# RIKEN-RCCS/EigenExa

Measured on AMD Instinct MI355X. Metric: eigen_sx full-solve throughput (reference flop model: 4/3 N^3 + D&C GEMM + 2 nvec N^2), higher is better.
Workload: dtype f64; 1 GPU; N=8192 random symmetric fp64 (counter-based R+R^T, seed 20240807), eigen_sx all eigenpairs, m_forward=64, m_backward=128; parallelism=1 GPU (1x1 grid)

## Files before the change

eigenexa_amd/csrc/api.hip:

```cpp
#include "eigx_context.h"
#include "eigx_comm.h"
#include "../../include/eigenexa_amd.h"
#include <cstring>

namespace eigx {
Context g_ctx;
}

using namespace eigx;

extern "C" {

int eigx_init(int device) {
  return eigx_init_multi(device, 0, 1, nullptr, 'C');
}

int eigx_get_device_count(void) {
  int ndev = 0;
  if (hipGetDeviceCount(&ndev) != hipSuccess) { (void)hipGetLastError(); return 0; }
  return ndev;
}

int eigx_get_rccl_unique_id(void* out128) {
  return comm_get_unique_id(out128);
// ... 245 lines not shown
int eigx_profile_read(double* out6) {
  if (!g_ctx.initialized) return EIGX_ERR_NOT_INITIALIZED;
  if (!out6) return EIGX_ERR_BAD_ARG;
  EIGX_HIP_CHECK(hipSetDevice(g_ctx.device));
  EIGX_HIP_CHECK(hipStreamSynchronize(g_ctx.stream));
  for (int q = 0; q < 6; ++q) out6[q] = 0.0;
  for (size_t q = 0; q < g_ctx.prof_kind.size(); ++q) {
    float ms = 0.f;
    EIGX_HIP_CHECK(hipEventElapsedTime(&ms, g_ctx.prof_ev[2 * q], g_ctx.prof_ev[2 * q + 1]));
    if (g_ctx.prof_kind[q] > 1) continue;
    const int k = g_ctx.prof_kind[q] ? 3 : 0;
    out6[k + 0] += 1.0;
    out6[k + 1] += g_ctx.prof_units[q];
    out6[k + 2] += 1e-3 * ms;
  }
  return EIGX_OK;
}

int eigx_profile_read_kinds(double* out, int nkinds) {
  if (!g_ctx.initialized) return EIGX_ERR_NOT_INITIALIZED;
  if (!out || nkinds < 1) return EIGX_ERR_BAD_ARG;
  EIGX_HIP_CHECK(hipSetDevice(g_ctx.device));
  EIGX_HIP_CHECK(hipStreamSynchronize(g_ctx.stream));
  for (int q = 0; q < 3 * nkinds; ++q) out[q] = 0.0;
  for (size_t q = 0; q < g_ctx.prof_kind.size(); ++q) {
    const int k = g_ctx.prof_kind[q];
    if (k < 0 || k >= nkinds) continue;
    float ms = 0.f;
    EIGX_HIP_CHECK(hipEventElapsedTime(&ms, g_ctx.prof_ev[2 * q], g_ctx.prof_ev[2 * q + 1]));
    out[3 * k + 0] += 1.0;
    out[3 * k + 1] += g_ctx.prof_units[q];
    out[3 * k + 2] += 1e-3 * ms;
  }
  return EIGX_OK;
}

int eigx_device_synchronize(void) {
  if (!g_ctx.initialized) return EIGX_ERR_NOT_INITIALIZED;
  EIGX_HIP_CHECK(hipSetDevice(g_ctx.device));
  EIGX_HIP_CHECK(hipDeviceSynchronize());
  return EIGX_OK;
}

void* eigx_malloc_dev(int64_t bytes) {
  if (!g_ctx.initialized) return nullptr;
  void* p = nullptr;
  if (hipMalloc(&p, (size_t)bytes) != hipSuccess) return nullptr;
  return p;
}
int eigx_free_dev(void* p) {
  if (p) EIGX_HIP_CHECK(hipFree(p));
  return EIGX_OK;
}
int eigx_memcpy_h2d(void* dst, const void* src, int64_t bytes) {
  EIGX_HIP_CHECK(hipMemcpy(dst, src, (size_t)bytes, hipMemcpyHostToDevice));
  return EIGX_OK;
}
int eigx_memcpy_d2h(void* dst, const void* src, int64_t bytes) {
  EIGX_HIP_CHECK(hipMemcpy(dst, src, (size_t)bytes, hipMemcpyDeviceToHost));
  return EIGX_OK;
}

int eigx_tune(int key, int value) {
  if (key == 0) return set_gemm_variant(value);
  if (key == 1) return set_bisect_threads(value);
  if (key == 2) return set_bt_q(value);
  if (key == 3 || key == 4 || key == 5 || key == 10 || key == 11) return set_reduce_knob(key, value);
  if (key == 12) return (value >= 0 && value <= 2) ? set_reduce_knob(key, value) : -1;
  if (key == 6) return set_gemm_cstream(value);
  if (key == 7) return value > 0 ? set_reduce_knob(key, value) : -1;
  if (key == 8) return set_dc_chunk(value);
  if (key == 9) return comm_set_bounce(value);
  if (key == 15) return set_dc_pipe(value);
  if (key == 16) return set_dc_batch(value);
  if (key == 17 || key == 18 || key == 19) return set_range_knob(key, value);
  if (key == 20) return set_tri_nb(value);
  if (key == 21) return set_batch_nmax(value);
  if (key == 22) return set_hbatch_nmax(value);
  if (key == 23) return set_gbatch_nmax(value);
  if (key == 24) return set_hgbatch_nmax(value);
  if (key == 25) return set_gemm_latec_kmax(value);
  if (key == 26) return set_batch_range_route(value);
  if (key == 27) return set_batch_range_accept(value);
  return -1;
}

int eigx_dgemm_dev(char opa, char opb, int m, int n, int k, double alpha, const double* a, int lda,
                   const double* b, int ldb, double beta, double* c, int ldc, int tri_upper) {
  if (!g_ctx.initialized) return EIGX_ERR_NOT_INITIALIZED;
  EIGX_HIP_CHECK(hipStreamSynchronize(nullptr));
  dgemm_dev(g_ctx.stream, opa, opb, m, n, k, alpha, a, lda, b, ldb, beta, c, ldc, tri_upper ? 1 : 0,
            &g_ctx.grid);
  EIGX_HIP_CHECK(hipStreamSynchronize(g_ctx.stream));
  return EIGX_OK;
}

int eigx_dgemm_gather_dev(char opa, char opb, int m, int n, int k, double alpha, const double* a, int lda,
                          const double* b, int ldb, double beta, double* c, int ldc, const int* kmap_a,
                          const int* kmap_b) {
  if (!g_ctx.initialized) return EIGX_ERR_NOT_INITIALIZED;
  EIGX_HIP_CHECK(hipStreamSynchronize(nullptr));
  dgemm_dev(g_ctx.stream, opa, opb, m, n, k, alpha, a, lda, b, ldb, beta, c, ldc, 0, nullptr, kmap_a, nullptr, 1, 0,
            0, 0, 1, 0, 0, 0, 1, 0, kmap_b);
  EIGX_HIP_CHECK(hipStreamSynchronize(g_ctx.stream));
  return EIGX_OK;
}

}
```

eigenexa_amd/csrc/dc.hip:

```cpp
#include "eigx_context.h"
#include "eigx_comm.h"
#include "../../include/eigenexa_amd.h"
#include <algorithm>
#include <cfloat>
#include <cstring>

namespace eigx {

namespace {

constexpr int LEAF = 32;

constexpr int LEAF_T = 64;
__global__ __launch_bounds__(LEAF_T) void jacobi_leaf_kernel(const double* __restrict__ d,
                                                             const double* __restrict__ e, int lde, int band,
                                                             const int* __restrict__ leaf_off,
                                                             const int* __restrict__ leaf_n, double* __restrict__ D,
                                                             double* __restrict__ Q, int ldq, int r0, int r1) {
  __shared__ double A[LEAF][LEAF + 1];
  __shared__ double V[LEAF][LEAF + 1];
  __shared__ double cs[LEAF / 2][2];
  __shared__ int pq[LEAF / 2][2];
  __shared__ int perm[LEAF];
  const int tid = threadIdx.x;
// ... 172 lines not shown
  const MergeDev M = md[blockIdx.z];
  const int K = M.K;
  if ((int)(blockIdx.x * 64) >= K || (int)(blockIdx.y * ZN_IC) >= K) return;
  const int i0 = blockIdx.y * ZN_IC;
  const int i1 = (i0 + ZN_IC < K) ? i0 + ZN_IC : K;
  {
    const int i = i0 + threadIdx.x;
    double y = 0.0;
    if (i < i1) {
      const double* col = Qa + (size_t)nd[M.off + i] * ldq;
      for (int t = 0; t < M.zr_n; ++t) y += M.zr_w[t] * col[M.zr_row[t]];
    }
    ys[threadIdx.x] = y;
  }
  __syncthreads();
  const int lane = threadIdx.x & 63, wave = threadIdx.x >> 6;
  const int j = blockIdx.x * 64 + lane;
  const bool act = j < K;
  const double* Sp = S + (size_t)M.off * lds + M.off + j;
  double acc = 0.0;
  if (act)
    for (int i = i0 + wave; i < i1; i += 4) acc += ys[i - i0] * Sp[(size_t)i * lds];
  part[wave][lane] = acc;
  __syncthreads();
  if (wave == 0 && act)
    zp[(size_t)blockIdx.y * ldn + M.off + j] = (part[0][lane] + part[1][lane]) + (part[2][lane] + part[3][lane]);
}
__global__ void znext2_kernel(const MergeDev* __restrict__ md, const int* __restrict__ dsrc, const double* __restrict__ Qa,
                              int ldq, const double* __restrict__ zp, int ldn, double* __restrict__ z) {
  const MergeDev M = md[blockIdx.y];
  const int jj = blockIdx.x * blockDim.x + threadIdx.x;
  if (jj >= M.nm) return;
  double v = 0.0;
  if (jj < M.K) {
    const int nch = (M.K + ZN_IC - 1) / ZN_IC;
    for (int c = 0; c < nch; ++c) v += zp[(size_t)c * ldn + M.off + jj];
  } else {
    const double* col = Qa + (size_t)dsrc[M.off + jj] * ldq;
    for (int t = 0; t < M.zr_n; ++t) v += M.zr_w[t] * col[M.zr_row[t]];
  }
  z[M.off + jj] = v;
}

__global__ void pack_rows_kernel(const double* __restrict__ Q, int ldq, int n, int r0, int nr, int rp,
                                 double* __restrict__ out) {
  const int j = blockIdx.y;
  for (int r = blockIdx.x * blockDim.x + threadIdx.x; r < rp; r += gridDim.x * blockDim.x)
    out[(size_t)j * rp + r] = (r < nr) ? Q[(size_t)j * ldq + r0 + r] : 0.0;
}
__global__ void unpack_rows_kernel(const double* __restrict__ in, int n, int rp, double* __restrict__ Q, int ldq) {
  const int j = blockIdx.y, q = blockIdx.z;
  const double* src = in + (size_t)q * rp * n + (size_t)j * rp;
  for (int r = blockIdx.x * blockDim.x + threadIdx.x; r < rp; r += gridDim.x * blockDim.x)
    if (q * rp + r < n) Q[(size_t)j * ldq + q * rp + r] = src[r];
}

template <int CTRL>
__device__ __forceinline__ double dc_dpp_add(double v) {
  const int lo2 = __builtin_amdgcn_update_dpp(0, __double2loint(v), CTRL, 0xf, 0xf, true);
  const int hi2 = __builtin_amdgcn_update_dpp(0, __double2hiint(v), CTRL, 0xf, 0xf, true);
  return v + __hiloint2double(hi2, lo2);
}

__device__ __forceinline__ double dc_swapadd16(double v) {
  const auto lo = __builtin_amdgcn_permlane16_swap(__double2loint(v), __double2loint(v), false, false);
  const auto hi = __builtin_amdgcn_permlane16_swap(__double2hiint(v), __double2hiint(v), false, false);
  return __hiloint2double(hi[0], lo[0]) + __hiloint2double(hi[1], lo[1]);
}

__device__ __forceinline__ double group8_sum(double v) {
  v = dc_dpp_add<0xB1>(v);
  v = dc_dpp_add<0x4E>(v);
  v = dc_dpp_add<0x141>(v);
  return v;
}

template <int LPR>
__device__ __forceinline__ double group_sum(double v) {
  v = group8_sum(v);
  if (LPR == 32) { v = dc_dpp_add<0x140>(v); v = dc_swapadd16(v); }
  return v;
}

template <int LPR>
__global__ __launch_bounds__(256) void secular_kernel(const MergeDev* __restrict__ md,
                                                      const double* __restrict__ dlam,
                                                      const double* __restrict__ wz, double* __restrict__ Dn,
                                                      double* __restrict__ S, int lds, int P, int rank,
                                                      double* __restrict__ sec, int nsec) {
  const MergeDev M = md[blockIdx.y];
  const int K = M.K;
  constexpr int RPW = 256 / LPR;
  __shared__ double so[RPW], stau[RPW];
  const int jbase = (P > 1) ? (int)((long)K * rank / P) : 0;
  const int jend = (P > 1) ? (int)((long)K * (rank + 1) / P) : K;
  if (jbase + (int)(blockIdx.x * RPW) >= jend) return;
  const int sub = threadIdx.x & (LPR - 1);
  const int jraw = jbase + blockIdx.x * RPW + threadIdx.x / LPR;
  const bool act = jraw < jend;
  const int j = act ? jraw : K - 1;
  const double* __restrict__ d = dlam + M.off;
  const double* __restrict__ z = wz + M.off;
  double* Sp = S + (size_t)M.off * lds + M.off;
  const double rho = M.rho, rhoinv = 1.0 / rho;
  const double eps = DBL_EPSILON / 2.0;
  if (K == 1) {
    if (threadIdx.x == 0) {
      const double t = rho * z[0] * z[0];
      if (sec) { sec[M.off] = d[0] + t; sec[nsec + M.off] = d[0]; sec[2 * nsec + M.off] = t; }
      else { Dn[M.off] = d[0] + t; Sp[0] = -t; }
    }
    return;
  }
  const bool last = (j == K - 1);
  const int jl = last ? K - 2 : j, jr = jl + 1;
  double origin, lo, hi, tau;
  {
    const double gap = last ? rho : d[j + 1] - d[j];
    const double base = last ? d[K - 1] : d[j], half = 0.5 * gap;
    double c = 0.0;
    for (int i = sub; i < K; i += LPR)
      if (i != jl && i != jr) c += z[i] * z[i] / ((d[i] - base) - half);
    c = group_sum<LPR>(c) + rhoinv;
    const double zl2 = z[jl] * z[jl], zr2 = z[jr] * z[jr];
    const double fmid = c + zl2 / ((d[jl] - base) - half) + zr2 / ((d[jr] - base) - half);
    int org;
    if (last) { org = K - 1; if (fmid <= 0.0) { lo = 0.5 * gap; hi = gap; } else { lo = 0.0; hi = 0.5 * gap; } }
    else if (fmid > 0.0) { org = j; lo = 0.0; hi = 0.5 * gap; }
    else { org = j + 1; lo = -0.5 * gap; hi = 0.0; }
    origin = d[org];
    const double dl = d[jl] - origin, dr = d[jr] - origin;
    const double qa = c, qb = -(c * (dl + dr) + zl2 + zr2), qc = c * dl * dr + zl2 * dr + zr2 * dl;
    tau = 0.5 * (lo + hi);
    const double disc = qb * qb - 4.0 * qa * qc;
    if (disc >= 0.0) {
      const double sq = sqrt(disc);
      const double qq = -0.5 * (qb + (qb >= 0.0 ? sq : -sq));
      const double r1 = (qa != 0.0) ? qq / qa : NAN, r2 = (qq != 0.0) ? qc / qq : NAN;
      if (r1 > lo && r1 < hi) tau = r1;
      else if (r2 > lo && r2 < hi) tau = r2;
    }
  }
  for (int iter = 0; iter < 100; ++iter) {
    double psi = 0.0, dpsi = 0.0, phi = 0.0, dphi = 0.0, err = 0.0;
    for (int i = sub; i < K; i += LPR) {
      const double t = z[i] / ((d[i] - origin) - tau);
      const double zt = z[i] * t, tt = t * t;
      if (i <= jl) { psi += zt; dpsi += tt; err += fabs(psi); }
      else { phi += zt; dphi += tt; err += fabs(phi); }
    }
    psi = group_sum<LPR>(psi); dpsi = group_sum<LPR>(dpsi);
    phi = group_sum<LPR>(phi); dphi = group_sum<LPR>(dphi);
    err = group_sum<LPR>(err);
    const double wv = rhoinv + phi + psi;
    err = 8.0 * (fabs(phi) + fabs(psi)) + err + 2.0 * rhoinv + fabs(tau) * (dpsi + dphi);
    if (fabs(wv) <= eps * err) break;
    if (wv < 0.0) lo = tau; else hi = tau;
    const double Dl = (d[jl] - origin) - tau, Dr = (d[jr] - origin) - tau;
    const double aa = (Dl + Dr) * wv - Dl * Dr * (dpsi + dphi);
    const double bb = Dl * Dr * wv;
    const double cc = wv - Dl * dpsi - Dr * dphi;
    double eta;
    {
      double disc = aa * aa - 4.0 * bb * cc;
      if (disc < 0.0) disc = 0.0;
      const double sq = sqrt(disc);
      if (cc == 0.0) eta = (aa != 0.0) ? bb / aa : 0.0;
      else if (aa <= 0.0) eta = (aa - sq) / (2.0 * cc);
      else eta = 2.0 * bb / (aa + sq);
    }
    if (wv * eta >= 0.0) eta = -wv / (dpsi + dphi);
    double tnew = tau + eta;
    if (!(tnew > lo && tnew < hi)) tnew = 0.5 * (lo + hi);
    if (tnew == tau) break;
    tau = tnew;
  }
  if (sec) {
    if (sub == 0 && act) { sec[M.off + j] = origin + tau; sec[nsec + M.off + j] = origin; sec[2 * nsec + M.off + j] = tau; }
    return;
  }
  if (sub == 0) { so[threadIdx.x / LPR] = origin; stau[threadIdx.x / LPR] = tau; if (act) Dn[M.off + j] = origin + tau; }
  __syncthreads();
  {
    const int r = threadIdx.x % RPW, ii = threadIdx.x / RPW;
    const int jr = blockIdx.x * RPW + r;
    if (jr < K) {
      const double o_ = so[r], t_ = stau[r];
      for (int i = ii; i < K; i += 256 / RPW) Sp[jr + (size_t)i * lds] = (d[i] - o_) - t_;
    }
  }
}

__global__ __launch_bounds__(256) void loewner_kernel(const MergeDev* __restrict__ md,
                                                      const double* __restrict__ dlam,
                                                      const double* __restrict__ wz, const double* __restrict__ S,
                                                      int lds, double* __restrict__ zh) {
  const MergeDev M = md[blockIdx.y];
  const int K = M.K;
  const int lane = threadIdx.x & 63;
  const int i = blockIdx.x * 4 + (threadIdx.x >> 6);
  if (i >= K) return;
  const double* d = dlam + M.off;
  const double* Sp = S + (size_t)M.off * lds + M.off + (size_t)i * lds;
  const double di = d[i];
  double prod = 1.0;
  for (int j = lane; j < K; j += 64) {
    const double num = -Sp[j];
    prod *= (j == i) ? num : num / (d[j] - di);
  }
  for (int o = 32; o > 0; o >>= 1) prod *= __shfl_xor(prod, o, 64);
  if (lane == 0) {
    const double v = sqrt(fabs(prod));
    zh[M.off + i] = (wz[M.off + i] >= 0.0) ? v : -v;
  }
}

constexpr int VEC_IC = 256;
__global__ __launch_bounds__(256) void vectors1_kernel(const MergeDev* __restrict__ md, const double* __restrict__ zh,
                                                       double* __restrict__ S, int lds, double* __restrict__ vnp,
                                                       int ldn) {
  __shared__ double part[4][64];
  const MergeDev M = md[blockIdx.z];
  const int K = M.K;
  if ((int)(blockIdx.x * 64) >= K || (int)(blockIdx.y * VEC_IC) >= K) return;
  const int lane = threadIdx.x & 63, wave = threadIdx.x >> 6;
  const int j = blockIdx.x * 64 + lane;
  const bool act = j < K;
  double* Sp = S + (size_t)M.off * lds + M.off + j;
  const double* zz = zh + M.off;
  const int i0 = blockIdx.y * VEC_IC;
  const int i1 = (i0 + VEC_IC < K) ? i0 + VEC_IC : K;
  double nrm = 0.0;
  if (act)
    for (int i = i0 + wave; i < i1; i += 4) {
      const double v = zz[i] / Sp[(size_t)i * lds];
      Sp[(size_t)i * lds] = v;
      nrm += v * v;
    }
  part[wave][lane] = nrm;
  __syncthreads();
  if (wave == 0 && act)
    vnp[(size_t)blockIdx.y * ldn + M.off + j] = (part[0][lane] + part[1][lane]) + (part[2][lane] + part[3][lane]);
}
__global__ __launch_bounds__(256) void vectors2_kernel(const MergeDev* __restrict__ md, double* __restrict__ S, int lds,
                                                       const double* __restrict__ vnp, int ldn) {
  const MergeDev M = md[blockIdx.z];
  const int K = M.K;
  if ((int)(blockIdx.x * 64) >= K || (int)(blockIdx.y * VEC_IC) >= K) return;
  const int lane = threadIdx.x & 63, wave = threadIdx.x >> 6;
  const int j = blockIdx.x * 64 + lane;
  if (j >= K) return;
  const int nch = (K + VEC_IC - 1) / VEC_IC;
  double nrm = 0.0;
  for (int c = 0; c < nch; ++c) nrm += vnp[(size_t)c * ldn + M.off + j];
  const double sc = 1.0 / sqrt(nrm);
  double* Sp = S + (size_t)M.off * lds + M.off + j;
  const int i0 = blockIdx.y * VEC_IC;
  const int i1 = (i0 + VEC_IC < K) ? i0 + VEC_IC : K;
  for (int i = i0 + wave; i < i1; i += 4) Sp[(size_t)i * lds] *= sc;
}

__global__ void scatter_lambda_kernel(const MergeDev* __restrict__ md, const double* __restrict__ sec, double* __restrict__ Dn) {
  const MergeDev M = md[blockIdx.y];
  const int j = blockIdx.x * blockDim.x + threadIdx.x;
  if (j < M.K) Dn[M.off + j] = sec[M.off + j];
}
__global__ __launch_bounds__(256) void loewner_mg_kernel(const MergeDev* __restrict__ md, const double* __restrict__ dlam,
                                                         const double* __restrict__ wz, const double* __restrict__ sec,
                                                         int nsec, double* __restrict__ zh) {
  const MergeDev M = md[blockIdx.y];
  const int K = M.K;
  const int lane = threadIdx.x & 63;
  const int i = blockIdx.x * 4 + (threadIdx.x >> 6);
  if (i >= K) return;
  const double* d = dlam + M.off;
  const double* org = sec + nsec + M.off;
  const double* tau = sec + 2 * nsec + M.off;
  const double di = d[i];
  double prod = 1.0;
  for (int j = lane; j < K; j += 64) {
    const double num = (org[j] - di) + tau[j];
    prod *= (j == i) ? num : num / (d[j] - di);
  }
  for (int o = 32; o > 0; o >>= 1) prod *= __shfl_xor(prod, o, 64);
  if (lane == 0) {
    const double v = sqrt(fabs(prod));
    zh[M.off + i] = (wz[M.off + i] >= 0.0) ? v : -v;
  }
}
__global__ __launch_bounds__(256) void vectors_mg_kernel(const MergeDev* __restrict__ md, int mi0, const double* __restrict__ dlam,
                                                         const double* __restrict__ zh, const double* __restrict__ sec, int nsec,
                                                         int j0, int j1, int compact, double* __restrict__ Sc, int ldsc) {
  __shared__ double part[4][64];
  const MergeDev M = md[mi0 + blockIdx.z];
  const int K = M.K;
  const int jhi = (j1 < K) ? j1 : K;
  const int lane = threadIdx.x & 63, wave = threadIdx.x >> 6;
  const int j = j0 + blockIdx.x * 64 + lane;
  if (j0 + (int)(blockIdx.x * 64) >= jhi) return;
  const bool act = j < jhi;
  const double* d = dlam + M.off;
  const double* zz = zh + M.off;
  const double oj = act ? sec[nsec + M.off + j] : 0.0, tj = act ? sec[2 * nsec + M.off + j] : 1.0;
  double nrm = 0.0;
  for (int i = wave; i < K; i += 4) {
    const double v = zz[i] / ((d[i] - oj) - tj);
    nrm += v * v;
  }
  part[wave][lane] = nrm;
  __syncthreads();
  const double sc = 1.0 / sqrt((part[0][lane] + part[1][lane]) + (part[2][lane] + part[3][lane]));
  if (!act) return;
  double* dst = Sc + (compact ? (size_t)M.off * ldsc : 0) + (j - j0);
  for (int i = wave; i < K; i += 4) dst[(size_t)i * ldsc] = zz[i] / ((d[i] - oj) - tj) * sc;
}

__global__ void pack_q_for_cols_kernel(const int* __restrict__ perm, const double* __restrict__ Q, int ldq, int r0, int nr,
                                       int rp, int zc, int nvec, double* __restrict__ send) {
  const int c = blockIdx.y, p = blockIdx.z;
  const int g = p * zc + c;
  if (c >= zc) return;
  double* dst = send + ((size_t)p * zc + c) * rp;
  if (g >= nvec) { for (int r = blockIdx.x * blockDim.x + threadIdx.x; r < rp; r += gridDim.x * blockDim.x) dst[r] = 0.0; return; }
  const double* src = Q + (size_t)perm[g] * ldq + r0;
  for (int r = blockIdx.x * blockDim.x + threadIdx.x; r < rp; r += gridDim.x * blockDim.x) dst[r] = (r < nr) ? src[r] : 0.0;
}
__global__ void unpack_cols_kernel(const double* __restrict__ recv, int rp, int zc, int n, double* __restrict__ Z, int ldz) {
  const int c = blockIdx.y, q = blockIdx.z;
  const double* src = recv + ((size_t)q * zc + c) * rp;
  for (int r = blockIdx.x * blockDim.x + threadIdx.x; r < rp; r += gridDim.x * blockDim.x)
    if (q * rp + r < n) Z[(size_t)c * ldz + q * rp + r] = __hip_atomic_load(src + r, __ATOMIC_RELAXED, __HIP_MEMORY_SCOPE_SYSTEM);
}

__global__ void copycols_kernel(const int* __restrict__ src, const int* __restrict__ dst,
                                const int* __restrict__ row0, const int* __restrict__ nrows,
                                const double* __restrict__ Qa, double* __restrict__ Qb, int ldq) {
  const int p = blockIdx.x;
  const double* s = Qa + (size_t)src[p] * ldq + row0[p];
  double* t = Qb + (size_t)dst[p] * ldq + row0[p];
  for (int r = threadIdx.x; r < nrows[p]; r += blockDim.x) t[r] = s[r];
}

__global__ void final_permute_kernel(const int* __restrict__ perm, const double* __restrict__ Q, int ldq, int n,
// ... 38 lines not shown

struct HostDC {
  int n, band, lde;
  std::vector<double> d, e;
  std::vector<Node> nodes;
  double& E(int i, int b) { return e[(size_t)(b - 1) * lde + i]; }

  int build(int off, int nn) {
    const int id = (int)nodes.size();
    nodes.push_back(Node());
    nodes[id].off = off; nodes[id].n = nn;
    if (nn <= LEAF) return id;
    const int n1 = nn / 2;
    nodes[id].n1 = n1;
    double c[4] = {0, 0, 0, 0}, sig[2] = {0, 0}, x[4] = {0, 0, 0, 0}, y[4] = {0, 0, 0, 0};
    for (int r = 0; r < band; ++r)
      for (int cc = r; cc < band; ++cc) {
        const int gi = off + n1 + r, gj = off + n1 - band + cc;
        c[r + band * cc] = E(gi, gi - gj);
      }
    svd2(band, c, sig, x, y);
    for (int k = 0; k < band; ++k) {
      for (int r = 0; r < band; ++r)
        for (int cc = 0; cc < band; ++cc) {
          const int i1 = off + n1 - band + r, j1 = off + n1 - band + cc;
          const double v1 = sig[k] * y[band * k + r] * y[band * k + cc];
          if (i1 == j1) d[i1] -= v1; else if (i1 < j1) E(j1, j1 - i1) -= v1;
          const int i2 = off + n1 + r, j2 = off + n1 + cc;
          const double v2 = sig[k] * x[band * k + r] * x[band * k + cc];
          if (i2 == j2) d[i2] -= v2; else if (i2 < j2) E(j2, j2 - i2) -= v2;
        }
      nodes[id].sig[k] = sig[k];
      for (int r = 0; r < band; ++r) {
        nodes[id].wv[k][r] = y[band * k + r];
        nodes[id].wv[k][band + r] = x[band * k + r];
      }
    }
    const int l = build(off, n1);
    const int r = build(off + n1, nn - n1);
    nodes[id].left = l; nodes[id].right = r;
    nodes[l].parent = id; nodes[r].parent = id;
    nodes[id].height = 1 + std::max(nodes[l].height, nodes[r].height);
    return id;
  }
};

void sort_index_runs(const double* d, int nm, std::vector<int>& idx, std::vector<int>& tmp, std::vector<int>& bounds) {
  idx.resize(nm);
  for (int i = 0; i < nm; ++i) idx[i] = i;
  bounds.clear();
  bounds.push_back(0);
  for (int i = 1; i < nm; ++i)
    if (d[i] < d[i - 1]) bounds.push_back(i);
  bounds.push_back(nm);
  auto cmp = [d](int a, int b) { return d[a] < d[b] || (d[a] == d[b] && a < b); };
  int nr = (int)bounds.size() - 1;
  if (nr > 16) { std::sort(idx.begin(), idx.end(), cmp); return; }
  tmp.resize(nm);
  while (nr > 1) {
    int w = 0;
    for (int r = 0; r < nr; r += 2) {
      if (r + 1 < nr)
        std::merge(idx.begin() + bounds[r], idx.begin() + bounds[r + 1], idx.begin() + bounds[r + 1], idx.begin() + bounds[r + 2],
                   tmp.begin() + bounds[r], cmp);
      else
        std::copy(idx.begin() + bounds[r], idx.begin() + bounds[r + 1], tmp.begin() + bounds[r]);
      bounds[w++] = bounds[r];
    }
    bounds[w] = nm;
    nr = w;
    idx.swap(tmp);
  }
}

}

int g_dc_pipe = 1, g_dc_batch = 1, g_dc_side_min = 1024;
int set_dc_pipe(int v) {
  const int old = g_dc_pipe;
  if (v >= 2) g_dc_side_min = v; else g_dc_pipe = v ? 1 : 0;
  return old;
}
int set_dc_batch(int v) { const int old = g_dc_batch; g_dc_batch = v ? 1 : 0; return old; }
int g_dc_chunk = 2048;
int set_dc_chunk(int v) {
  const int old = g_dc_chunk;
  if (v >= 64 && v <= 2048 && v % 64 == 0) g_dc_chunk = v;
  return old;
}

void band_dc_prepare(Context& ctx, int n) {
  const int P = ctx.grid.nranks;
  const int ldq = (P > 1) ? pad_ld((n + P - 1) / P + 2) : pad_ld(n);
  double* Qa = ctx.pool.get_t<double>("dc.Qa", (size_t)ldq * n);
  double* Qb = ctx.pool.get_t<double>("dc.Qb", (size_t)ldq * n);
  EIGX_HIP_CHECK(hipMemsetAsync(Qa, 0, (size_t)ldq * n * 8, ctx.side_stream));
  EIGX_HIP_CHECK(hipMemsetAsync(Qb, 0, (size_t)ldq * n * 8, ctx.side_stream));
  EIGX_HIP_CHECK(hipEventRecord(ctx.dc_ev, ctx.side_stream));
  ctx.dc_zero_n = n; ctx.dc_zero_qa = Qa; ctx.dc_zero_qb = Qb;
}

void band_dc_dev(Context& ctx, int n, int nvec, const double* d_dev, const double* e_dev, int lde, int band,
                 double* w_dev, double* z_dev, int ldz, const std::function<void()>& side_work) {
  hipStream_t st = ctx.stream;
  const double eps = DBL_EPSILON / 2.0;
  const int P = ctx.grid.nranks;
  const int rp = (n + P - 1) / P;
  const int r0 = P > 1 ? std::min(n, ctx.grid.rank * rp) : 0;
  const int r1 = P > 1 ? std::min(n, r0 + rp) : n;
  auto clip = [&](int lo, int hi, int& a, int& b) { a = std::max(lo, r0); b = std::min(hi, r1); return b > a; };
  HostDC H;
  H.n = n; H.band = band; H.lde = lde;
  H.d.resize(n);
  H.e.resize((size_t)lde * band);
  EIGX_HIP_CHECK(hipMemcpyAsync(H.d.data(), d_dev, (size_t)n * 8, hipMemcpyDeviceToHost, st));
  EIGX_HIP_CHECK(hipMemcpyAsync(H.e.data(), e_dev, (size_t)lde * band * 8, hipMemcpyDeviceToHost, st));
  EIGX_HIP_CHECK(hipStreamSynchronize(st));
  double nrm = 0.0;
  for (int i = 0; i < n; ++i) {
    nrm = std::max(nrm, fabs(H.d[i]));
    for (int b = 1; b <= band; ++b) if (i >= b) nrm = std::max(nrm, fabs(H.E(i, b)));
  }
  const double scl = nrm > 0.0 ? 1.0 / nrm : 1.0;
  for (int i = 0; i < n; ++i) {
    H.d[i] *= scl;
    for (int b = 1; b <= band; ++b) H.E(i, b) = (i >= b) ? H.E(i, b) * scl : 0.0;
  }
  H.nodes.reserve(2 * (n / (LEAF / 2) + 2));
  const int root = H.build(0, n);
  const int maxh = H.nodes[root].height;

  const bool pipe = (P == 1) && g_dc_pipe;
  const int ldq = (P > 1) ? pad_ld(rp + 2) : pad_ld(n);
  double* Qa_base = ctx.pool.get_t<double>("dc.Qa", (size_t)ldq * n);
  double* Qb_base = ctx.pool.get_t<double>("dc.Qb", (size_t)ldq * n);
  double* Qa = Qa_base - r0;
  double* Qb = Qb_base - r0;
  const int SCW = g_dc_chunk;
  const int lds_mg = SCW;
  double* Sbuf[2];
  Sbuf[0] = ctx.pool.get_t<double>("dc.S", (P > 1) ? (size_t)n * SCW + 64 : (size_t)ldq * n);
  Sbuf[1] = pipe ? ctx.pool.get_t<double>("dc.S2", (size_t)ldq * n) : Sbuf[0];
  double* sec = (P > 1) ? ctx.pool.get_t<double>("dc.sec", (size_t)3 * n) : nullptr;
  double* dd = ctx.pool.get_t<double>("dc.d", (size_t)n);
  double* de = ctx.pool.get_t<double>("dc.e", (size_t)lde * band);
  double* zh = ctx.pool.get_t<double>("dc.zh", (size_t)n);
  double* vnp = ctx.pool.get_t<double>("dc.vnp", (size_t)n * ((n + VEC_IC - 1) / VEC_IC + 1));
  double* zp = pipe ? ctx.pool.get_t<double>("dc.zp", (size_t)n * ((n + ZN_IC - 1) / ZN_IC + 1)) : nullptr;
  const int maxmerge = n / (LEAF / 2) + 8;
  int* leafinfo = ctx.pool.get_t<int>("dc.leaf", (size_t)2 * maxmerge);
  int* perm_dev = ctx.pool.get_t<int>("dc.perm", (size_t)n);
  int* iota_dev = ctx.pool.get_t<int>("dc.iota", (size_t)n);
  struct Arena {
    char *dev, *host;
    MergeDev *md_dev, *md_h;
    GemmBatch *gb_dev, *gb_h;
    int *nd_dev, *nd_h, *rpj_dev, *rpj_h, *rjj_dev, *rjj_h, *cps_dev, *cps_h, *cpd_dev, *cpd_h, *cpr_dev, *cpr_h, *cpn_dev, *cpn_h;
    int *topA_dev, *topA_h, *topB_dev, *topB_h, *botA_dev, *botA_h, *botB_dev, *botB_h, *dsrc_dev, *dsrc_h;
    double *dlam, *dl_h, *wz, *wz_h, *rc_dev, *rc_h, *rs_dev, *rs_h, *Dcur, *Dh, *zbuf, *zhost;
  } ar[2];
  const size_t npad = ((size_t)n + 7) / 8 * 8;
  const size_t md_bytes = ((size_t)maxmerge * sizeof(MergeDev) + 63) / 64 * 64;
  const size_t gb_bytes = ((size_t)2 * maxmerge * sizeof(GemmBatch) + 63) / 64 * 64;
  const size_t up_bytes = md_bytes + gb_bytes + 12 * npad * sizeof(int) + 5 * npad * sizeof(double);
  const size_t arena_bytes = up_bytes + npad * sizeof(double);
  const size_t down_off = up_bytes - npad * 8;
  {
    char* dev_all = (char*)ctx.pool.get("dc.arena", 2 * arena_bytes);
    char* host_all = (char*)ctx.pool.get_host("dc.arena", 2 * arena_bytes);
    memset(host_all, 0, 2 * arena_bytes);
    for (int q = 0; q < 2; ++q) {
      Arena& A = ar[q];
      A.dev = dev_all + q * arena_bytes;
      A.host = host_all + q * arena_bytes;
      size_t pos = 0;
      auto carve = [&](size_t bytes, void* pd, void* ph) {
        *(char**)pd = A.dev + pos; *(char**)ph = A.host + pos; pos += bytes;
      };
      carve(md_bytes, &A.md_dev, &A.md_h);
      carve(gb_bytes, &A.gb_dev, &A.gb_h);
      carve(npad * 4, &A.nd_dev, &A.nd_h);
      carve(npad * 4, &A.rpj_dev, &A.rpj_h);  carve(npad * 4, &A.rjj_dev, &A.rjj_h);
      carve(npad * 4, &A.cps_dev, &A.cps_h);  carve(npad * 4, &A.cpd_dev, &A.cpd_h);
      carve(npad * 4, &A.cpr_dev, &A.cpr_h);  carve(npad * 4, &A.cpn_dev, &A.cpn_h);
      carve(npad * 4, &A.topA_dev, &A.topA_h); carve(npad * 4, &A.topB_dev, &A.topB_h);
      carve(npad * 4, &A.botA_dev, &A.botA_h); carve(npad * 4, &A.botB_dev, &A.botB_h);
      carve(npad * 4, &A.dsrc_dev, &A.dsrc_h);
      carve(npad * 8, &A.dlam, &A.dl_h);  carve(npad * 8, &A.wz, &A.wz_h);
      carve(npad * 8, &A.rc_dev, &A.rc_h); carve(npad * 8, &A.rs_dev, &A.rs_h);
      carve(npad * 8, &A.Dcur, &A.Dh);    carve(npad * 8, &A.zbuf, &A.zhost);
    }
  }
  MergeDev* md_h2 = (MergeDev*)ctx.pool.get_host("dc.md2", md_bytes);

  EIGX_HIP_CHECK(hipMemcpyAsync(dd, H.d.data(), (size_t)n * 8, hipMemcpyHostToDevice, st));
  EIGX_HIP_CHECK(hipMemcpyAsync(de, H.e.data(), (size_t)lde * band * 8, hipMemcpyHostToDevice, st));
  if (ctx.dc_zero_n == n && ctx.dc_zero_qa == Qa_base && ctx.dc_zero_qb == Qb_base) {
    EIGX_HIP_CHECK(hipStreamWaitEvent(st, ctx.dc_ev, 0));
  } else {
    EIGX_HIP_CHECK(hipMemsetAsync(Qa_base, 0, (size_t)ldq * n * 8, st));
    EIGX_HIP_CHECK(hipMemsetAsync(Qb_base, 0, (size_t)ldq * n * 8, st));
  }
  ctx.dc_zero_n = 0;
  {
    std::vector<int> iota(n);
    for (int q = 0; q < n; ++q) iota[q] = q;
    EIGX_HIP_CHECK(hipMemcpyAsync(iota_dev, iota.data(), (size_t)n * 4, hipMemcpyHostToDevice, st));
    EIGX_HIP_CHECK(hipStreamSynchronize(st));
  }

  double* Dfinal = ar[1].Dcur;
  {
    std::vector<int> lo, ln;
    for (const Node& nd : H.nodes)
      if (nd.left < 0) { lo.push_back(nd.off); ln.push_back(nd.n); }
    const int nl = (int)lo.size();
    std::vector<int> both(lo);
    both.insert(both.end(), ln.begin(), ln.end());
    EIGX_HIP_CHECK(hipMemcpyAsync(leafinfo, both.data(), (size_t)2 * nl * 4, hipMemcpyHostToDevice, st));
    EIGX_HIP_CHECK(hipStreamSynchronize(st));
    hipLaunchKernelGGL(jacobi_leaf_kernel, dim3(nl), dim3(LEAF_T), 0, st, dd, de, lde, band, leafinfo, leafinfo + nl,
                       Dfinal, Qa, ldq, r0, r1);
  }
  bool side_done = false;
  auto run_side_work = [&] {
    if (side_done || !side_work) return;
// ... 133 lines not shown
            }
            if (pj >= 0) { C.nd_h[off + K] = off + pj; ++K; }
          } else {
            for (int i = 0; i < nm; ++i) defl.push_back(i);
          }
        } else {
          for (int i = 0; i < nm; ++i) defl.push_back(i);
        }
        M.rot_end = nrot;
        for (int t = 0; t < K; ++t) { C.dl_h[off + t] = dloc[C.nd_h[off + t] - off]; C.wz_h[off + t] = zloc[C.nd_h[off + t] - off]; }
        for (int t = 1; t < K; ++t) {
          int u = t;
          while (u > 0 && C.dl_h[off + u] < C.dl_h[off + u - 1]) {
            std::swap(C.dl_h[off + u], C.dl_h[off + u - 1]);
            std::swap(C.wz_h[off + u], C.wz_h[off + u - 1]);
            std::swap(C.nd_h[off + u], C.nd_h[off + u - 1]);
            --u;
          }
        }
        M.K = K;
        M.rho = rho;
        {
          int nt_ = 0, nb_ = 0;
          for (int t = 0; t < K; ++t) {
            const int col = C.nd_h[off + t], ty = ctype[col];
            if (ty != 2) { C.topA_h[off + nt_] = col; C.topB_h[off + nt_] = t; ++nt_; }
            if (ty != 1) { C.botA_h[off + nb_] = col; C.botB_h[off + nb_] = t; ++nb_; }
          }
          ktop[q] = nt_; kbot[q] = nb_;
        }
        for (size_t t = 0; t < defl.size(); ++t) {
          const int src = off + defl[t], dst = off + K + (int)t;
          int ca, cb;
          if (clip(off, off + nm, ca, cb)) {
            C.cps_h[ncopy] = src; C.cpd_h[ncopy] = dst; C.cpr_h[ncopy] = ca; C.cpn_h[ncopy] = cb - ca;
            ++ncopy;
          }
          C.dsrc_h[dst] = src;
          C.Dh[dst] = dloc[defl[t]];
        }
        for (int t = 0; t < K; ++t) C.Dh[off + t] = 0.0;
      }
      int maxK = 0;
      for (const MergeDev& M : mds) maxK = std::max(maxK, M.K);
      const unsigned nmg = (unsigned)ids.size();
      hipStream_t sb = (pipe && maxnm > g_dc_side_min) ? ctx.dc_stream : st;
      const bool batched = (P == 1) && g_dc_batch && maxK > 0 && mds.size() > 1 &&
                           (long)ceil_div(maxnm, 128) * ceil_div(maxK, 128) < 192;
      int nbatch = 0, bmaxM = 0;
      if (batched) {
        const int bot_shift = (int)(C.botA_dev - C.topA_dev);
        for (size_t q = 0; q < mds.size(); ++q) {
          const MergeDev& M = mds[q];
          if (M.K <= 0) continue;
          auto add = [&](int row0, int rows, int kk, int offKA, int offKB) {
            if (rows <= 0) return;
            GemmBatch& B = C.gb_h[nbatch++];
            B.M = rows; B.N = M.K; B.K = kk; B.pad = 0;
            B.offA = row0; B.offB = (long)M.off * ldq + M.off; B.offC = (long)M.off * ldq + row0;
            B.offKA = offKA; B.offKB = offKB;
            bmaxM = std::max(bmaxM, rows);
          };
          if (k == 0) {
            add(M.off, M.n1, ktop[q], M.off, M.off);
            add(M.off + M.n1, M.nm - M.n1, kbot[q], M.off + bot_shift, M.off + bot_shift);
            gemm_flops += 2.0 * (double)M.K * ((double)M.n1 * ktop[q] + (double)(M.nm - M.n1) * kbot[q]);
          } else {
            add(M.off, M.nm, M.K, M.off, 0);
            gemm_flops += 2.0 * M.nm * (double)M.K * M.K;
          }
        }
      }
      const double tt2 = trace ? now_s() : 0.0;
      double t_gemm_enq = 0.0;
      memcpy(C.md_h, mds.data(), mds.size() * sizeof(MergeDev));
      EIGX_HIP_CHECK(hipMemcpyAsync(C.dev, C.host, up_bytes, hipMemcpyHostToDevice, sb));
      const bool mg = P > 1;
      const bool compact = mg && maxnm <= lds_mg;
      if (maxK > 0) {
        if (mg) {
          const int kmx = maxK / P + 2;
          EIGX_HIP_CHECK(hipMemsetAsync(sec, 0, (size_t)3 * n * 8, st));
          if (maxK >= 512)
            hipLaunchKernelGGL(secular_kernel<32>, dim3((kmx + 7) / 8, nmg), dim3(256), 0, st, C.md_dev, C.dlam, C.wz, C.Dcur, S, ldq, P,
                               ctx.grid.rank, sec, n);
          else
            hipLaunchKernelGGL(secular_kernel<8>, dim3((kmx + 31) / 32, nmg), dim3(256), 0, st, C.md_dev, C.dlam, C.wz, C.Dcur, S, ldq, P,
                               ctx.grid.rank, sec, n);
          comm_allreduce_sum(ctx, COMM_WORLD, sec, (size_t)3 * n, st);
          hipLaunchKernelGGL(scatter_lambda_kernel, dim3((maxK + 255) / 256, nmg), dim3(256), 0, st, C.md_dev, sec, C.Dcur);
          hipLaunchKernelGGL(loewner_mg_kernel, dim3((maxK + 3) / 4, nmg), dim3(256), 0, st, C.md_dev, C.dlam, C.wz, sec, n, zh);
          if (compact)
            hipLaunchKernelGGL(vectors_mg_kernel, dim3((maxK + 63) / 64, 1, nmg), dim3(256), 0, st, C.md_dev, 0, C.dlam, zh, sec, n, 0,
                               maxK, 1, S, lds_mg);
        } else {
          if (maxK >= 512)
            hipLaunchKernelGGL(secular_kernel<32>, dim3((maxK + 7) / 8, nmg), dim3(256), 0, sb, C.md_dev, C.dlam, C.wz, C.Dcur, S, ldq, 1, 0,
                               (double*)nullptr, 0);
          else
            hipLaunchKernelGGL(secular_kernel<8>, dim3((maxK + 31) / 32, nmg), dim3(256), 0, sb, C.md_dev, C.dlam, C.wz, C.Dcur, S, ldq, 1, 0,
                               (double*)nullptr, 0);
          hipLaunchKernelGGL(loewner_kernel, dim3((maxK + 3) / 4, nmg), dim3(256), 0, sb, C.md_dev, C.dlam, C.wz, S, ldq, zh);
          const dim3 vg((maxK + 63) / 64, (maxK + VEC_IC - 1) / VEC_IC, nmg);
          hipLaunchKernelGGL(vectors1_kernel, vg, dim3(256), 0, sb, C.md_dev, zh, S, ldq, vnp, n);
          hipLaunchKernelGGL(vectors2_kernel, vg, dim3(256), 0, sb, C.md_dev, S, ldq, vnp, n);
        }
      }
      if (sb != st) {
        EIGX_HIP_CHECK(hipEventRecord(ctx.dc_b_ev, sb));
        EIGX_HIP_CHECK(hipStreamWaitEvent(st, ctx.dc_b_ev, 0));
      }
      if (pipe && pi + 1 == passes.size()) {
        EIGX_HIP_CHECK(hipMemcpyAsync(V.Dh, C.Dcur, (size_t)n * 8, hipMemcpyDeviceToHost, sb));
        EIGX_HIP_CHECK(hipEventRecord(ctx.dc_z_ev, sb));
        early_final = V.Dh;
      }
      if (nrot > 0)
        hipLaunchKernelGGL(rotate_kernel, dim3((maxnm + 255) / 256, nmg), dim3(256), 0, st, C.md_dev,
                           C.rpj_dev, C.rjj_dev, C.rc_dev, C.rs_dev, Qa, ldq, r0, r1);
      if (z_ahead) {
        if (maxK > 0)
          hipLaunchKernelGGL(znext1_kernel, dim3((maxK + 63) / 64, (maxK + ZN_IC - 1) / ZN_IC, nmg), dim3(256), 0, st, C.md_dev,
                             C.nd_dev, Qa, ldq, S, ldq, zp, n);
        hipLaunchKernelGGL(znext2_kernel, dim3((maxnm + 255) / 256, nmg), dim3(256), 0, st, C.md_dev, C.dsrc_dev, Qa, ldq, zp, n,
                           C.zbuf);
        EIGX_HIP_CHECK(hipMemcpyAsync(C.host + down_off, C.dev + down_off, 2 * npad * 8, hipMemcpyDeviceToHost, st));
        EIGX_HIP_CHECK(hipEventRecord(ctx.dc_z_ev, st));
        z_ready = true;
      }
      if (pi + 1 == passes.size()) run_side_work();
      if (maxK > 0) {
        const bool fan = mds.size() > 1 && !(mg && !compact) && !batched;
        if (fan) {
          EIGX_HIP_CHECK(hipEventRecord(ctx.aux_ev[Context::kAux], st));
          for (int q = 0; q < Context::kAux; ++q) EIGX_HIP_CHECK(hipStreamWaitEvent(ctx.aux[q], ctx.aux_ev[Context::kAux], 0));
        }
        int rr = 0;
        const double tg0 = trace ? now_s() : 0.0;
        if (batched) {
          if (k == 0)
            dgemm_gather_batch_dev(st, C.gb_dev, nbatch, bmaxM, maxK, Qa, ldq, S, ldq, Qb, ldq, C.topA_dev, C.topB_dev);
          else
            dgemm_gather_batch_dev(st, C.gb_dev, nbatch, bmaxM, maxK, Qa, ldq, S, ldq, Qb, ldq, C.nd_dev, iota_dev);
        } else
        for (size_t q = 0; q < mds.size(); ++q) {
          const MergeDev& M = mds[q];
          if (M.K <= 0) continue;
          const bool chunked = mg && !compact;
          int cwq = M.K;
          if (chunked) { cwq = (int)(((size_t)n * SCW / (size_t)M.K) / 64 * 64); if (cwq > M.K) cwq = M.K; if (cwq < 64) cwq = 64; }
          for (int j0 = 0; j0 < M.K; j0 += cwq) {
          const int cw = (M.K - j0 < cwq) ? M.K - j0 : cwq;
          const int ldsb = mg ? (chunked ? ((cw + 1) & ~1) : lds_mg) : ldq;
          const double* Sb = mg ? (chunked ? S : S + (size_t)M.off * lds_mg) : S + (size_t)M.off * ldq + M.off;
          if (chunked) {
            hipLaunchKernelGGL(vectors_mg_kernel, dim3((cw + 63) / 64, 1, 1), dim3(256), 0, st, C.md_dev, (int)q, C.dlam, zh, sec, n, j0,
                               j0 + cw, 0, S, ldsb);
          }
          double* Cb = Qb + (size_t)(M.off + j0) * ldq + M.off;
          if (k == 0) {
            hipStream_t g1 = fan ? ctx.aux[rr++ % Context::kAux] : st;
            hipStream_t g2 = fan ? ctx.aux[rr++ % Context::kAux] : ((mds.size() == 1 && !chunked) ? ctx.aux[0] : st);
            if (!fan && g2 != st) {
              EIGX_HIP_CHECK(hipEventRecord(ctx.aux_ev[Context::kAux], st));
              EIGX_HIP_CHECK(hipStreamWaitEvent(g2, ctx.aux_ev[Context::kAux], 0));
            }
            int ga, gb;
            if (clip(M.off, M.off + M.n1, ga, gb))
              dgemm_dev(g1, 'N', 'T', gb - ga, cw, ktop[q], 1.0, Qa + ga, ldq, Sb, ldsb, 0.0, Cb + (ga - M.off), ldq, 0,
                        nullptr, C.topA_dev + M.off, nullptr, 1, 0, 0, 0, 1, 0, 0, 0, 1, 0, C.topB_dev + M.off);
            if (clip(M.off + M.n1, M.off + M.nm, ga, gb))
              dgemm_dev(g2, 'N', 'T', gb - ga, cw, kbot[q], 1.0, Qa + ga, ldq, Sb, ldsb, 0.0, Cb + (ga - M.off), ldq, 0,
                        nullptr, C.botA_dev + M.off, nullptr, 1, 0, 0, 0, 1, 0, 0, 0, 1, 0, C.botB_dev + M.off);
            if (!fan && g2 != st) {
              EIGX_HIP_CHECK(hipEventRecord(ctx.aux_ev[0], g2));
              EIGX_HIP_CHECK(hipStreamWaitEvent(st, ctx.aux_ev[0], 0));
            }
            gemm_flops += 2.0 * (double)cw * ((double)M.n1 * ktop[q] + (double)(M.nm - M.n1) * kbot[q]);
          } else {
            hipStream_t gs = fan ? ctx.aux[rr++ % Context::kAux] : st;
            int ga, gb;
            if (clip(M.off, M.off + M.nm, ga, gb))
              dgemm_dev(gs, 'N', 'T', gb - ga, cw, M.K, 1.0, Qa + ga, ldq, Sb, ldsb, 0.0, Cb + (ga - M.off), ldq, 0,
                        nullptr, C.nd_dev + M.off, nullptr, 1, 0, 0, 0, 1, 0, 0, 0, 1, 0, iota_dev);
// ... 87 lines not shown
```

eigenexa_amd/csrc/eigx_common.h:

```cpp
#pragma once
#include <hip/hip_runtime.h>
#include <cstdio>
#include <cstdlib>
#include <cstdint>
#include <cmath>
#include <vector>
#include <ctime>
#include <chrono>

#define EIGX_HIP_CHECK(expr)                                                        \
  do {                                                                              \
    hipError_t _e = (expr);                                                         \
    if (_e != hipSuccess) {                                                         \
      fprintf(stderr, "[eigx] HIP error %s at %s:%d: %s\n", hipGetErrorName(_e),    \
              __FILE__, __LINE__, hipGetErrorString(_e));                           \
      abort();                                                                      \
    }                                                                               \
  } while (0)

namespace eigx {

typedef double d4_t __attribute__((ext_vector_type(4)));

struct Grid {
// ... 11 lines not shown
  if (m < 512) return l + (512 - m);
  if (m > 1536) return l + (2048 - m) + 512;
  return l;
}
static inline int pad_ld(int n) {
  static const int extra = [] { const char* e = getenv("EIGX_LD_EXTRA"); return e ? atoi(e) : 0; }();
  int l = (n + 31) / 32;
  if (l * 32 >= 2048) return hbm_ld(l * 32) + extra;
  if ((l & 1) == 0) ++l;
  return l * 32 + extra;
}
static inline int64_t ceil_div64(int64_t a, int64_t b) { return (a + b - 1) / b; }

static inline int local_count(int n, int P, int p) { return n > p ? (n - p + P - 1) / P : 0; }
static inline int numroc(int n, int nb, int p, int P) {
  const int nblocks = n / nb;
  int cnt = (nblocks / P) * nb;
  const int extra = nblocks % P;
  if (p < extra) cnt += nb;
  else if (p == extra) cnt += n % nb;
  return cnt;
}

inline double now_s() {
  return std::chrono::duration<double>(std::chrono::steady_clock::now().time_since_epoch()).count();
}

struct SolveRequest {
  char mode;
  int nvec;
  bool want_vec;
};
inline char upper_case(char c) { return (c >= 'a' && c <= 'z') ? (char)(c - 'a' + 'A') : c; }
inline SolveRequest normalize_request(int n, int nvec, char mode) {
  mode = upper_case(mode);
  if (nvec == 0) mode = 'N';
  if (nvec < 0) nvec = -nvec;
  if (nvec > n) nvec = n;
  return SolveRequest{mode, nvec, mode != 'N'};
}


__global__ void fill_kernel(double* p, size_t n, double v);
__global__ void fill_vec_kernel(double* __restrict__ w, int n, double v);
__global__ void scale_vec_kernel(double* __restrict__ w, int n, double s);

void dgemm_dev(hipStream_t stream, char opA, char opB, int M, int N, int K, double alpha,
               const double* A, int lda, const double* B, int ldb, double beta, double* C, int ldc,
               int tri_mode = 0, const Grid* g = nullptr, const int* kmapA = nullptr,
               const int* cmapC = nullptr, int batch = 1, long strideA = 0, long strideB = 0, long strideC = 0,
               int batch2 = 1, long strideA2 = 0, long strideB2 = 0, long strideC2 = 0, int ownP = 1,
               int ownp = 0, const int* kmapB = nullptr, int tn_lo = 0, int tn_hi = 0x7fffffff);

int gemm_tri2_launch_tiles(int M, int N, const Grid& g, int tn_lo, int tn_hi);

struct GemmBatch {
  int M, N, K, pad;
  long offA, offB, offC;
  int offKA, offKB;
};
void dgemm_gather_batch_dev(hipStream_t stream, const GemmBatch* tab_dev, int nbatch, int maxM, int maxN,
                            const double* A, int lda, const double* B, int ldb, double* C, int ldc,
                            const int* kmapA, const int* kmapB);

inline void stage_trace(int rank, const char* what, long detail = -1) {
  static const bool on = getenv("EIGX_TRACE_STAGES") != nullptr;
  if (!on) return;
  timespec ts;
  clock_gettime(CLOCK_MONOTONIC, &ts);
  if (detail >= 0) fprintf(stderr, "[eigx stage] rank %d t=%.3f %s %ld\n", rank, ts.tv_sec % 100000 + ts.tv_nsec * 1e-9, what, detail);
  else fprintf(stderr, "[eigx stage] rank %d t=%.3f %s\n", rank, ts.tv_sec % 100000 + ts.tv_nsec * 1e-9, what);
  fflush(stderr);
}

int set_gemm_variant(int v);
int set_gemm_cstream(int v);
int set_gemm_latec_kmax(int v);
int set_bisect_threads(int v);
int set_bt_q(int v);
int set_reduce_knob(int key, int v);
int set_dc_chunk(int v);
int set_dc_pipe(int v);
int set_dc_batch(int v);
int set_batch_nmax(int v);
int set_hbatch_nmax(int v);
int get_batch_nmax();
int get_hbatch_nmax();
int set_gbatch_nmax(int v);
int set_hgbatch_nmax(int v);
int get_gbatch_nmax();
int set_batch_range_route(int v);
int set_batch_range_accept(int v);

}
```

Measured before the change: 19450 GFLOP/s.

## Add chained secular/Loewner/vector path for single-GPU D&C merges

For a single GPU, the secular solver now writes compact (lambda, origin, tau) triples instead of the full difference matrix S, which removes the shared-memory staging, sync and large S write. It then uses the multi-group Loewner kernel and new vnorm/vstore kernels that recompute vector entries on the fly and write normalized eigenvectors straight into S. The path is on by default through a new knob and needs an extra small sec buffer. In exchange, the divisions are recomputed in two passes.

```diff
diff --git a/eigenexa_amd/csrc/api.hip b/eigenexa_amd/csrc/api.hip
--- a/eigenexa_amd/csrc/api.hip
+++ b/eigenexa_amd/csrc/api.hip
@@ -351,6 +351,7 @@
   if (key == 25) return set_gemm_latec_kmax(value);
   if (key == 26) return set_batch_range_route(value);
   if (key == 27) return set_batch_range_accept(value);
+  if (key == 28) return set_dc_chain(value);
   return -1;
 }
 
diff --git a/eigenexa_amd/csrc/dc.hip b/eigenexa_amd/csrc/dc.hip
--- a/eigenexa_amd/csrc/dc.hip
+++ b/eigenexa_amd/csrc/dc.hip
@@ -278,7 +278,7 @@
   return v;
 }
 
-template <int LPR>
+template <int LPR, bool STORE_S>
 __global__ __launch_bounds__(256) void secular_kernel(const MergeDev* __restrict__ md,
                                                       const double* __restrict__ dlam,
                                                       const double* __restrict__ wz, double* __restrict__ Dn,
@@ -287,7 +287,6 @@
   const MergeDev M = md[blockIdx.y];
   const int K = M.K;
   constexpr int RPW = 256 / LPR;
-  __shared__ double so[RPW], stau[RPW];
   const int jbase = (P > 1) ? (int)((long)K * rank / P) : 0;
   const int jend = (P > 1) ? (int)((long)K * (rank + 1) / P) : K;
   if (jbase + (int)(blockIdx.x * RPW) >= jend) return;
@@ -303,8 +302,11 @@
   if (K == 1) {
     if (threadIdx.x == 0) {
       const double t = rho * z[0] * z[0];
-      if (sec) { sec[M.off] = d[0] + t; sec[nsec + M.off] = d[0]; sec[2 * nsec + M.off] = t; }
-      else { Dn[M.off] = d[0] + t; Sp[0] = -t; }
+      if (STORE_S) { Dn[M.off] = d[0] + t; Sp[0] = -t; }
+      else {
+        sec[M.off] = d[0] + t; sec[nsec + M.off] = d[0]; sec[2 * nsec + M.off] = t;
+        if (P == 1) Dn[M.off] = d[0] + t;
+      }
     }
     return;
   }
@@ -371,13 +373,15 @@
     if (tnew == tau) break;
     tau = tnew;
   }
-  if (sec) {
-    if (sub == 0 && act) { sec[M.off + j] = origin + tau; sec[nsec + M.off + j] = origin; sec[2 * nsec + M.off + j] = tau; }
-    return;
-  }
-  if (sub == 0) { so[threadIdx.x / LPR] = origin; stau[threadIdx.x / LPR] = tau; if (act) Dn[M.off + j] = origin + tau; }
-  __syncthreads();
-  {
+  if constexpr (!STORE_S) {
+    if (sub == 0 && act) {
+      sec[M.off + j] = origin + tau; sec[nsec + M.off + j] = origin; sec[2 * nsec + M.off + j] = tau;
+      if (P == 1) Dn[M.off + j] = origin + tau;
+    }
+  } else {
+    __shared__ double so[RPW], stau[RPW];
+    if (sub == 0) { so[threadIdx.x / LPR] = origin; stau[threadIdx.x / LPR] = tau; if (act) Dn[M.off + j] = origin + tau; }
+    __syncthreads();
     const int r = threadIdx.x % RPW, ii = threadIdx.x / RPW;
     const int jr = blockIdx.x * RPW + r;
     if (jr < K) {
@@ -455,6 +459,56 @@
   const int i1 = (i0 + VEC_IC < K) ? i0 + VEC_IC : K;
   for (int i = i0 + wave; i < i1; i += 4) Sp[(size_t)i * lds] *= sc;
 }
+__global__ __launch_bounds__(256) void vnorm_kernel(const MergeDev* __restrict__ md, const double* __restrict__ dlam,
+                                                    const double* __restrict__ zh, const double* __restrict__ sec, int nsec,
+                                                    double* __restrict__ vnp, int ldn) {
+  __shared__ double part[4][64];
+  const MergeDev M = md[blockIdx.z];
+  const int K = M.K;
+  if ((int)(blockIdx.x * 64) >= K || (int)(blockIdx.y * VEC_IC) >= K) return;
+  const int lane = threadIdx.x & 63, wave = threadIdx.x >> 6;
+  const int j = blockIdx.x * 64 + lane;
+  const bool act = j < K;
+  const double* d = dlam + M.off;
+  const double* zz = zh + M.off;
+  const double oj = act ? sec[nsec + M.off + j] : 0.0, tj = act ? sec[2 * nsec + M.off + j] : 1.0;
+  const int i0 = blockIdx.y * VEC_IC;
+  const int i1 = (i0 + VEC_IC < K) ? i0 + VEC_IC : K;
+  double nrm = 0.0;
+  if (act)
+    for (int i = i0 + wave; i < i1; i += 4) {
+      const double v = zz[i] / ((d[i] - oj) - tj);
+      nrm += v * v;
+    }
+  part[wave][lane] = nrm;
+  __syncthreads();
+  if (wave == 0 && act)
+    vnp[(size_t)blockIdx.y * ldn + M.off + j] = (part[0][lane] + part[1][lane]) + (part[2][lane] + part[3][lane]);
+}
+__global__ __launch_bounds__(256) void vstore_kernel(const MergeDev* __restrict__ md, const double* __restrict__ dlam,
+                                                     const double* __restrict__ zh, const double* __restrict__ sec, int nsec,
+                                                     const double* __restrict__ vnp, int ldn, double* __restrict__ S, int lds) {
+  const MergeDev M = md[blockIdx.z];
+  const int K = M.K;
+  if ((int)(blockIdx.x * 64) >= K || (int)(blockIdx.y * VEC_IC) >= K) return;
+  const int lane = threadIdx.x & 63, wave = threadIdx.x >> 6;
+  const int j = blockIdx.x * 64 + lane;
+  if (j >= K) return;
+  const int nch = (K + VEC_IC - 1) / VEC_IC;
+  double nrm = 0.0;
+  for (int c = 0; c < nch; ++c) nrm += vnp[(size_t)c * ldn + M.off + j];
+  const double sc = 1.0 / sqrt(nrm);
+  const double* d = dlam + M.off;
+  const double* zz = zh + M.off;
+  const double oj = sec[nsec + M.off + j], tj = sec[2 * nsec + M.off + j];
+  double* Sp = S + (size_t)M.off * lds + M.off + j;
+  const int i0 = blockIdx.y * VEC_IC;
+  const int i1 = (i0 + VEC_IC < K) ? i0 + VEC_IC : K;
+  for (int i = i0 + wave; i < i1; i += 4) {
+    const double v = zz[i] / ((d[i] - oj) - tj);
+    Sp[(size_t)i * lds] = v * sc;
+  }
+}
 
 __global__ void scatter_lambda_kernel(const MergeDev* __restrict__ md, const double* __restrict__ sec, double* __restrict__ Dn) {
   const MergeDev M = md[blockIdx.y];
@@ -659,6 +713,13 @@
   return old;
 }
 int set_dc_batch(int v) { const int old = g_dc_batch; g_dc_batch = v ? 1 : 0; return old; }
+int g_dc_chain = 1;
+int set_dc_chain(int v) {
+  if (v != 0 && v != 1) return -1;
+  const int old = g_dc_chain;
+  g_dc_chain = v;
+  return old;
+}
 int g_dc_chunk = 2048;
 int set_dc_chunk(int v) {
   const int old = g_dc_chunk;
@@ -718,7 +779,7 @@
   double* Sbuf[2];
   Sbuf[0] = ctx.pool.get_t<double>("dc.S", (P > 1) ? (size_t)n * SCW + 64 : (size_t)ldq * n);
   Sbuf[1] = pipe ? ctx.pool.get_t<double>("dc.S2", (size_t)ldq * n) : Sbuf[0];
-  double* sec = (P > 1) ? ctx.pool.get_t<double>("dc.sec", (size_t)3 * n) : nullptr;
+  double* sec = (P > 1 || g_dc_chain) ? ctx.pool.get_t<double>("dc.sec", (size_t)3 * n) : nullptr;
   double* dd = ctx.pool.get_t<double>("dc.d", (size_t)n);
   double* de = ctx.pool.get_t<double>("dc.e", (size_t)lde * band);
   double* zh = ctx.pool.get_t<double>("dc.zh", (size_t)n);
@@ -1018,10 +1079,10 @@
           const int kmx = maxK / P + 2;
           EIGX_HIP_CHECK(hipMemsetAsync(sec, 0, (size_t)3 * n * 8, st));
           if (maxK >= 512)
-            hipLaunchKernelGGL(secular_kernel<32>, dim3((kmx + 7) / 8, nmg), dim3(256), 0, st, C.md_dev, C.dlam, C.wz, C.Dcur, S, ldq, P,
+            hipLaunchKernelGGL((secular_kernel<32, false>), dim3((kmx + 7) / 8, nmg), dim3(256), 0, st, C.md_dev, C.dlam, C.wz, C.Dcur, S, ldq, P,
                                ctx.grid.rank, sec, n);
           else
-            hipLaunchKernelGGL(secular_kernel<8>, dim3((kmx + 31) / 32, nmg), dim3(256), 0, st, C.md_dev, C.dlam, C.wz, C.Dcur, S, ldq, P,
+            hipLaunchKernelGGL((secular_kernel<8, false>), dim3((kmx + 31) / 32, nmg), dim3(256), 0, st, C.md_dev, C.dlam, C.wz, C.Dcur, S, ldq, P,
                                ctx.grid.rank, sec, n);
           comm_allreduce_sum(ctx, COMM_WORLD, sec, (size_t)3 * n, st);
           hipLaunchKernelGGL(scatter_lambda_kernel, dim3((maxK + 255) / 256, nmg), dim3(256), 0, st, C.md_dev, sec, C.Dcur);
@@ -1029,13 +1090,24 @@
           if (compact)
             hipLaunchKernelGGL(vectors_mg_kernel, dim3((maxK + 63) / 64, 1, nmg), dim3(256), 0, st, C.md_dev, 0, C.dlam, zh, sec, n, 0,
                                maxK, 1, S, lds_mg);
+        } else if (g_dc_chain) {
+          if (maxK >= 512)
+            hipLaunchKernelGGL((secular_kernel<32, false>), dim3((maxK + 7) / 8, nmg), dim3(256), 0, sb, C.md_dev, C.dlam, C.wz, C.Dcur, S,
+                               ldq, 1, 0, sec, n);
+          else
+            hipLaunchKernelGGL((secular_kernel<8, false>), dim3((maxK + 31) / 32, nmg), dim3(256), 0, sb, C.md_dev, C.dlam, C.wz, C.Dcur, S,
+                               ldq, 1, 0, sec, n);
+          hipLaunchKernelGGL(loewner_mg_kernel, dim3((maxK + 3) / 4, nmg), dim3(256), 0, sb, C.md_dev, C.dlam, C.wz, sec, n, zh);
+          const dim3 vg((maxK + 63) / 64, (maxK + VEC_IC - 1) / VEC_IC, nmg);
+          hipLaunchKernelGGL(vnorm_kernel, vg, dim3(256), 0, sb, C.md_dev, C.dlam, zh, sec, n, vnp, n);
+          hipLaunchKernelGGL(vstore_kernel, vg, dim3(256), 0, sb, C.md_dev, C.dlam, zh, sec, n, vnp, n, S, ldq);
         } else {
           if (maxK >= 512)
-            hipLaunchKernelGGL(secular_kernel<32>, dim3((maxK + 7) / 8, nmg), dim3(256), 0, sb, C.md_dev, C.dlam, C.wz, C.Dcur, S, ldq, 1, 0,
-                               (double*)nullptr, 0);
+            hipLaunchKernelGGL((secular_kernel<32, true>), dim3((maxK + 7) / 8, nmg), dim3(256), 0, sb, C.md_dev, C.dlam, C.wz, C.Dcur, S,
+                               ldq, 1, 0, (double*)nullptr, 0);
           else
-            hipLaunchKernelGGL(secular_kernel<8>, dim3((maxK + 31) / 32, nmg), dim3(256), 0, sb, C.md_dev, C.dlam, C.wz, C.Dcur, S, ldq, 1, 0,
-                               (double*)nullptr, 0);
+            hipLaunchKernelGGL((secular_kernel<8, true>), dim3((maxK + 31) / 32, nmg), dim3(256), 0, sb, C.md_dev, C.dlam, C.wz, C.Dcur, S,
+                               ldq, 1, 0, (double*)nullptr, 0);
           hipLaunchKernelGGL(loewner_kernel, dim3((maxK + 3) / 4, nmg), dim3(256), 0, sb, C.md_dev, C.dlam, C.wz, S, ldq, zh);
           const dim3 vg((maxK + 63) / 64, (maxK + VEC_IC - 1) / VEC_IC, nmg);
           hipLaunchKernelGGL(vectors1_kernel, vg, dim3(256), 0, sb, C.md_dev, zh, S, ldq, vnp, n);
diff --git a/eigenexa_amd/csrc/eigx_common.h b/eigenexa_amd/csrc/eigx_common.h
--- a/eigenexa_amd/csrc/eigx_common.h
+++ b/eigenexa_amd/csrc/eigx_common.h
@@ -117,6 +117,7 @@
 int set_dc_chunk(int v);
 int set_dc_pipe(int v);
 int set_dc_batch(int v);
+int set_dc_chain(int v);
 int set_batch_nmax(int v);
 int set_hbatch_nmax(int v);
 int get_batch_nmax();
```

Result: no change. 19510 GFLOP/s, median of 6 (+0.3%).
